# HBioquant/DiffBindFR

Hardware: AMD Instinct MI355X
Metric: poses_per_sec (higher is better)
Workload: dtype f32

## Files before the change

### diffbindfr_amd/csrc/convz.hip

```cpp
#include <cstdio>
#include <cstdlib>
#include <type_traits>

#include "common.h"

typedef float f32x4 __attribute__((ext_vector_type(4)));
typedef float f32x2 __attribute__((ext_vector_type(2)));
typedef _Float16 f16x8 __attribute__((ext_vector_type(8)));
typedef _Float16 f16x4 __attribute__((ext_vector_type(4)));
typedef _Float16 f16x2 __attribute__((ext_vector_type(2)));
typedef unsigned u32x4 __attribute__((ext_vector_type(4)));
typedef unsigned u32x2 __attribute__((ext_vector_type(2)));

#define CH_TILE_BYTES 9280
#define CH_TAIL_OFF 8192
#define CH_BIAS_OFF 9216

#define CZ_VSTRIDE 2064
#define CZ_CB (8 * CZ_VSTRIDE)
#define CZ_NCB 2
#define CZ_TILE (CZ_NCB * CZ_CB)
#define CZ_KPB 1
#define CZ_BUF (CZ_KPB * CZ_TILE)
#define CZ_ZBYTES (2 * CZ_BUF)
#define CZ_NHL 2
#define CZ_WAVE_FLOATS (32 * 12 + 32 + 32 + 32 + 32 + 32 + CZ_MAXSEG * 16 + 24 * 64 + CZ_NHL * 256)
#ifndef CZ_PRIO
#define CZ_PRIO 1
#endif
#if CZ_PRIO
#define CZ_SETPRIO(x) __builtin_amdgcn_s_setprio(x)
#else
#define CZ_SETPRIO(x)
#endif
#ifndef CZ_FETCH_AT
#define CZ_FETCH_AT 4
#endif
#ifndef CZ_PF_KT
#define CZ_PF_KT 7
#endif
#define CZ_ZSCALE (-20)

__device__ __forceinline__ void cz_split2(float x0, float x1, unsigned& hi, unsigned& lo) {
  const f16x2 h = __builtin_convertvector((f32x2){x0, x1}, f16x2);
  const f16x2 l = __builtin_convertvector((f32x2){x0 - (float)h[0], x1 - (float)h[1]}, f16x2);
  hi = __builtin_bit_cast(unsigned, h);
  lo = __builtin_bit_cast(unsigned, l);
}
__device__ __forceinline__ float cz_wave_max(float v) {
#pragma unroll
  for (int o = 1; o < 64; o <<= 1) v = fmaxf(v, __shfl_xor(v, o));
  return v;
}

__device__ __forceinline__ int cz_lane_here() {
  int l = __builtin_amdgcn_mbcnt_hi(~0u, __builtin_amdgcn_mbcnt_lo(~0u, 0u));
  asm volatile("" : "+v"(l));
  return l;
}

template <int I, int N, typename F>
__device__ __forceinline__ void cz_static_for(F&& f) {
  if constexpr (I < N) { f(std::integral_constant<int, I>{}); cz_static_for<I + 1, N>(f); }
}

template <int NW, int ABL = 0>
__global__ __launch_bounds__(64 * NW, 2) void k_convz(ConvZArgs a) {
  constexpr int KT = 9;
  extern __shared__ __attribute__((aligned(16))) float lds[];
  const int tid = threadIdx.x, lane = tid & 63, wave = __builtin_amdgcn_readfirstlane(tid >> 6);
  const int n = lane & 15, g = lane >> 4;
  char* zb = reinterpret_cast<char*>(lds);
  float* wl = lds + CZ_ZBYTES / 4 + wave * CZ_WAVE_FLOATS;
  float* w_sh = wl;
  float* w_sa = wl + 32 * 12;
  float* w_ua = w_sa + 32;
  int* w_row = reinterpret_cast<int*>(w_ua + 32);
  int* w_seg = w_row + 32;
  int* w_first = w_seg + 32;
  unsigned* w_mask = reinterpret_cast<unsigned*>(w_first + 32);
  float* w_xs = reinterpret_cast<float*>(w_mask + CZ_MAXSEG * 16);
  u32x4* w_hl = reinterpret_cast<u32x4*>(w_xs + 24 * 64);
  int* b_nseg = reinterpret_cast<int*>(lds + CZ_ZBYTES / 4 + NW * CZ_WAVE_FLOATS);
  int* b_col_edge = b_nseg + NW;
  float* b_col_inv = reinterpret_cast<float*>(b_col_edge + 16 * CZ_NCB);
  unsigned* b_cdesc = reinterpret_cast<unsigned*>(b_col_inv + 16 * CZ_NCB);

  int tr_n = 0;
  auto stamp = [&](int tag) {
    if constexpr ((ABL & 128) != 0) {
      if (a.dbg && blockIdx.x == 0 && lane == 0 && tr_n < 1000) {
        unsigned long long* t = reinterpret_cast<unsigned long long*>(a.dbg) + wave * 1024;
        t[tr_n++] = (__builtin_amdgcn_s_memtime() << 8) | (unsigned)tag;
      }
    }
  };
  int nch[4] = {0, 0, 0, 0}, nu[4] = {0, 0, 0, 0};
#pragma unroll
  for (int c = 0; c < 4; ++c)
    if (c < a.n_conv) {
      const ConvZDesc& d = a.c[c];
      nch[c] = min(*d.n_chunks, d.max_chunks);
      nu[c] = (nch[c] + NW - 1) / NW;
    }
  const int N = nu[0] + nu[1] + nu[2] + nu[3];
  for (int unit = blockIdx.x; unit < N; unit += gridDim.x) {
    int c = 0, ul = unit;
    if (ul >= nu[0]) { ul -= nu[0]; c = 1; if (ul >= nu[1]) { ul -= nu[1]; c = 2; if (ul >= nu[2]) { ul -= nu[2]; c = 3; } } }
    const ConvZDesc& d = a.c[c];
    const ConvZ& W = d.w;
    const int E = min(*d.n_edges, d.max_edges);
    unsigned cd_t = 0u;
    if (tid < (W.ct0[W.n_io - 1] + W.nct[W.n_io - 1]) * 16) cd_t = W.cdesc[tid];
    const int ch = ul * NW + wave;
    int es = 0, len = 0, gidx = 0;
    if (ch < nch[c]) {
      es = d.chunk_es[ch];
      const int gl = d.chunk_gl[ch];
      gidx = gl >> 6;
      len = min(min(gl & 63, 32), max(E - es, 0));
    }
    __syncthreads();
    if (unit != (int)blockIdx.x) tr_n = 1000;
    stamp(1);
    const int sl = lane & 31;
    const bool have = len > 0;
    const int e_sl = have ? es + min(sl, len - 1) : 0;
    const int tgt_ld = d.tgt[e_sl], gth_ld = d.gth[e_sl];
    float s_l[9];
    {
      const float* sp = d.sh + (size_t)e_sl * SH_LD;
#pragma unroll
      for (int k = 0; k < 9; ++k) s_l[k] = sp[k];
    }
    const float xmax_g = d.xmax ? d.xmax[gidx] : 0.f;
    int i1_t[2], i2_t[2];
    f32x4 Ba_t[2][9];
#pragma unroll
    for (int et = 0; et < 2; ++et) {
      const int e = have ? es + min(16 * et + n, len - 1) : 0;
      i1_t[et] = d.idx1[e];
      i2_t[et] = d.idx2[e];
      const float* r0 = d.emb + (size_t)e * NS;
#pragma unroll
      for (int s4 = 0; s4 < 3; ++s4) Ba_t[et][s4] = *reinterpret_cast<const f32x4*>(r0 + 16 * s4 + 4 * g);
    }
    const int tgt_l = have ? tgt_ld : 0, gth_l = have ? gth_ld : 0;
    const int tgt_prev = __shfl_up(tgt_l, 1);
    const bool is_first = lane < 32 && sl < len && (sl == 0 || tgt_l != tgt_prev);
    const unsigned long long bal = __ballot(is_first);
    const unsigned firsts = (unsigned)bal;
    const int nseg = min(__popc(firsts), CZ_MAXSEG);
    const int seg_l = (sl < len) ? __popc(firsts & (0xffffffffu >> (31 - sl))) - 1 : -1;
    if (lane < 32) {
      w_row[sl] = gth_l * d.ldx;
      w_seg[sl] = seg_l;
      if (is_first) w_first[seg_l] = sl;
#pragma unroll
      for (int k = 0; k < 9; ++k) w_sh[sl * 12 + k] = have ? s_l[k] : 0.f;
      w_sh[sl * 12 + 9] = w_sh[sl * 12 + 10] = w_sh[sl * 12 + 11] = 0.f;
    }
    if (lane == 0) b_nseg[wave] = nseg;
    if (tid < CZ_MAXCT * 16) b_cdesc[tid] = cd_t;
    float xmx = 0.f, smx = 0.f;
    if (have) {
      if (d.xmax) xmx = xmax_g;
      else {
        const float* xr = d.x + (size_t)gth_l * d.ldx;
        const int d4 = d.ldx >> 2;
        for (int j = lane >> 5; j < d4; j += 2) {
          const f32x4 v = *reinterpret_cast<const f32x4*>(xr + 4 * j);
          xmx = fmaxf(fmaxf(xmx, fmaxf(fabsf(v[0]), fabsf(v[1]))), fmaxf(fabsf(v[2]), fabsf(v[3])));
        }
      }
      if (lane < 32) {
#pragma unroll
        for (int k = 0; k < 9; ++k) smx = fmaxf(smx, fabsf(s_l[k]));
      }
    }
    xmx = cz_wave_max(xmx); smx = cz_wave_max(smx);
    int ey = 0;
    if (xmx > 0.f && smx > 0.f) ey = max(-100, min(100, 13 - __builtin_amdgcn_frexp_expf(xmx) - __builtin_amdgcn_frexp_expf(smx)));
    ey = __builtin_amdgcn_readfirstlane(ey);
    const float sY = __builtin_amdgcn_ldexpf(1.f, ey);

    stamp(2);
    u32x4 Hh[CZ_NKT][2];
    int eh = 0;
    {
      const __amdgpu_buffer_rsrc_t rW1 = __builtin_amdgcn_make_buffer_rsrc((void*)W.W1h, 0, KT * CH_TILE_BYTES, 0x00020000);
      u32x4 Ah[2][2][4];
      u32x4 Atc[2];
      const int vW = lane * 16;
      u32x4 F[3][2];
      auto ldF = [&](auto ic) {
        constexpr int i = decltype(ic)::value, m = i / 5, sx = i % 5;
        if constexpr (sx < 4) {
          F[i % 3][0] = __builtin_bit_cast(u32x4, __builtin_amdgcn_raw_buffer_load_b128(rW1, vW, m * CH_TILE_BYTES + sx * 1024, 0));
          F[i % 3][1] = __builtin_bit_cast(u32x4, __builtin_amdgcn_raw_buffer_load_b128(rW1, vW, m * CH_TILE_BYTES + (4 + sx) * 1024, 0));
        } else {
          F[i % 3][0] = __builtin_bit_cast(u32x4, __builtin_amdgcn_raw_buffer_load_b128(rW1, vW, m * CH_TILE_BYTES + CH_TAIL_OFF, 0));
          F[i % 3][1][0] = __builtin_amdgcn_raw_buffer_load_b32(rW1, n * 4, m * CH_TILE_BYTES + CH_BIAS_OFF, 0);
        }
      };
#pragma unroll
      for (int et = 0; et < 2; ++et) {
        const float* r1 = d.tab1 + (size_t)i1_t[et] * d.ld1;
        const float* r2 = d.tab2 + (size_t)i2_t[et] * d.ld2;
#pragma unroll
        for (int s4 = 3; s4 < KT; ++s4) Ba_t[et][s4] = *reinterpret_cast<const f32x4*>((s4 < 6 ? r1 : r2) + 16 * (s4 % 3) + 4 * g);
      }
      ldF(std::integral_constant<int, 0>{});
      ldF(std::integral_constant<int, 1>{});
#pragma unroll
      for (int et = 0; et < 2; ++et) {
        const int slot = 16 * et + n;
        f32x4 Ba[KT];
        float amx = 0.f;
#pragma unroll
        for (int s4 = 0; s4 < KT; ++s4) {
          Ba[s4] = have ? Ba_t[et][s4] : (f32x4){0.f, 0.f, 0.f, 0.f};
#pragma unroll
          for (int q = 0; q < 4; ++q) amx = fmaxf(amx, fabsf(Ba[s4][q]));
        }
        amx = fmaxf(amx, __shfl_xor(amx, 16));
        amx = fmaxf(amx, __shfl_xor(amx, 32));
        const int ja = max(-14, __builtin_amdgcn_frexp_expf(amx));
        const float sa = __builtin_amdgcn_ldexpf(1.f, 15 - ja);
        if (g == 0) { w_sa[slot] = sa; w_ua[slot] = __builtin_amdgcn_ldexpf(1.f, ja - 15); }
#pragma unroll
        for (int s4 = 0; s4 < KT; ++s4) {
          unsigned hi0, lo0, hi1, lo1;
          cz_split2(Ba[s4][0] * sa, Ba[s4][1] * sa, hi0, lo0);
          cz_split2(Ba[s4][2] * sa, Ba[s4][3] * sa, hi1, lo1);
          if (s4 < 8) {
            Ah[et][0][s4 >> 1][2 * (s4 & 1)] = hi0; Ah[et][0][s4 >> 1][2 * (s4 & 1) + 1] = hi1;
            Ah[et][1][s4 >> 1][2 * (s4 & 1)] = lo0; Ah[et][1][s4 >> 1][2 * (s4 & 1) + 1] = lo1;
          } else {
            Atc[et] = (u32x4){lo0, lo1, hi0, hi1};
          }
        }
      }
      __builtin_amdgcn_wave_barrier();
      f32x4 sar[2], uar[2];
#pragma unroll
      for (int et = 0; et < 2; ++et) {
        sar[et] = *reinterpret_cast<const f32x4*>(w_sa + 16 * et + 4 * g);
        uar[et] = *reinterpret_cast<const f32x4*>(w_ua + 16 * et + 4 * g);
      }
      float Hf[KT][2][4];
      float hmx = 0.f;
      f32x4 acc[2];
      cz_static_for<0, 5 * KT>([&](auto ic) {
        constexpr int i = decltype(ic)::value, m = i / 5, sx = i % 5;
        if constexpr (i + 2 < 5 * KT) ldF(std::integral_constant<int, (i + 2 < 5 * KT ? i + 2 : 0)>{});
        if constexpr (sx == 0) { acc[0] = (f32x4){0.f, 0.f, 0.f, 0.f}; acc[1] = (f32x4){0.f, 0.f, 0.f, 0.f}; }
        if constexpr (sx < 4) {
          const f16x8 whi = __builtin_bit_cast(f16x8, F[i % 3][0]), wlo = __builtin_bit_cast(f16x8, F[i % 3][1]);
#pragma unroll
          for (int et = 0; et < 2; ++et) {
            acc[et] = __builtin_amdgcn_mfma_f32_16x16x32_f16(__builtin_bit_cast(f16x8, Ah[et][1][sx]), whi, acc[et], 0, 0, 0);
            acc[et] = __builtin_amdgcn_mfma_f32_16x16x32_f16(__builtin_bit_cast(f16x8, Ah[et][0][sx]), wlo, acc[et], 0, 0, 0);
            acc[et] = __builtin_amdgcn_mfma_f32_16x16x32_f16(__builtin_bit_cast(f16x8, Ah[et][0][sx]), whi, acc[et], 0, 0, 0);
          }
        } else {
          const u32x4 wt = F[i % 3][0];
          const f16x8 wf = __builtin_bit_cast(f16x8, wt);
          const f16x8 wh = __builtin_bit_cast(f16x8, (u32x4){wt[0], wt[1], 0u, 0u});
          const float bias = __builtin_bit_cast(float, F[i % 3][1][0]);
          const float w1r = W.W1rinv ? W.W1rinv[16 * m + n] : 1.f;
#pragma unroll
          for (int et = 0; et < 2; ++et) {
            acc[et] = __builtin_amdgcn_mfma_f32_16x16x32_f16(__builtin_bit_cast(f16x8, Atc[et]), wf, acc[et], 0, 0, 0);
            acc[et] = __builtin_amdgcn_mfma_f32_16x16x32_f16(__builtin_bit_cast(f16x8, (u32x4){Atc[et][2], Atc[et][3], 0u, 0u}), wh, acc[et], 0, 0, 0);
          }
#pragma unroll
          for (int et = 0; et < 2; ++et)
#pragma unroll
            for (int q = 0; q < 4; ++q) {
              const float v = fmaxf(acc[et][q] + bias * sar[et][q], 0.f) * (uar[et][q] * w1r);
              Hf[m][et][q] = v;
              hmx = fmaxf(hmx, v);
            }
        }
      });
      if (!(ABL & 128) && a.dbg && unit == 0 && wave == 0) {
        const float k1i = __builtin_amdgcn_ldexpf(1.f, -W.k1);
#pragma unroll
        for (int m = 0; m < KT; ++m)
#pragma unroll
          for (int et = 0; et < 2; ++et)
#pragma unroll
            for (int q = 0; q < 4; ++q) a.dbg[(16 * et + 4 * g + q) * 144 + 16 * m + n] = Hf[m][et][q] * k1i;
      }
      hmx = cz_wave_max(hmx);
      eh = max(hmx > 0.f ? __builtin_amdgcn_frexp_expf(hmx) : W.k1, W.k1);
      eh = min(eh, W.k1 + 100);
      const float sH = __builtin_amdgcn_ldexpf(1.f, 15 - eh);
#pragma unroll
      for (int m = 0; m < KT; ++m) {
        unsigned h0, l0, h1, l1, h2, l2, h3, l3;
        cz_split2(Hf[m][0][0] * sH, Hf[m][0][1] * sH, h0, l0);
        cz_split2(Hf[m][0][2] * sH, Hf[m][0][3] * sH, h1, l1);
        cz_split2(Hf[m][1][0] * sH, Hf[m][1][1] * sH, h2, l2);
        cz_split2(Hf[m][1][2] * sH, Hf[m][1][3] * sH, h3, l3);
        Hh[m][0] = (u32x4){h0, h1, h2, h3};
        if (m < CZ_NHL) w_hl[m * 64 + lane] = (u32x4){l0, l1, l2, l3};
        else Hh[m][1] = (u32x4){l0, l1, l2, l3};
      }
    }
    const int ephi = 15 - eh + W.k1;
    {
      const _Float16 ph = (_Float16)__builtin_amdgcn_ldexpf(1.f, ephi);
      const unsigned short pb = __builtin_bit_cast(unsigned short, ph);
      u32x4 hb = {0u, 0u, 0u, 0u};
      if (n == 0) {
#pragma unroll
        for (int t = 0; t < 8; ++t) {
          const int slot = t < 4 ? 4 * g + t : 16 + 4 * g + (t - 4);
          if (slot < len) hb[t >> 1] |= (unsigned)pb << (16 * (t & 1));
        }
      }
      Hh[KT][0] = hb;
      Hh[KT][1] = (u32x4){0u, 0u, 0u, 0u};
    }
    stamp(3);
    {
      const int j = lane >> 4, gg = (lane >> 2) & 3, r = lane & 3, t0 = 2 * r;
      const int s0 = t0 < 4 ? 4 * gg + t0 : 16 + 4 * gg + (t0 - 4);
      w_mask[lane] = (w_seg[s0] == j ? 0x0000ffffu : 0u) | (w_seg[s0 + 1] == j ? 0xffff0000u : 0u);
    }
    __builtin_amdgcn_wave_barrier();
    __syncthreads();
    int cbase = 0, total = 0;
#pragma unroll
    for (int v = 0; v < NW; ++v) { const int c = b_nseg[v]; if (v < wave) cbase += c; total += c; }
    cbase = __builtin_amdgcn_readfirstlane(cbase); total = __builtin_amdgcn_readfirstlane(total);
    const int nseg_u = __builtin_amdgcn_readfirstlane(nseg);
    const int ncb = (total + 15) >> 4;
    const float col_inv = __builtin_amdgcn_ldexpf(1.f, -CZ_ZSCALE - ey - ephi);
    const float zs = __builtin_amdgcn_ldexpf(1.f, CZ_ZSCALE);
    if (ABL & 32) continue;
    for (int c = tid; c < 16 * CZ_NCB; c += 64 * NW) b_col_edge[c] = -1;
    __syncthreads();
    if (lane < nseg_u) {
      b_col_edge[cbase + lane] = es + w_first[lane];
      b_col_inv[cbase + lane] = col_inv;
    }
    char* za[CZ_MAXSEG];
    {
      char* zw0 = zb + (n & 7) * CZ_VSTRIDE + g * 512 + (n >> 3) * 256;
#pragma unroll
      for (int j = 0; j < CZ_MAXSEG; ++j) {
        const int col = cbase + j;
        za[j] = j < nseg_u ? zw0 + (col >> 4) * CZ_CB + (col & 15) * 16 : zw0 + CZ_CB + 15 * 16;
      }
    }
    long long n_mfma = 2 * KT * 14;
    for (int io = 0; io < W.n_io; ++io) {
      n_mfma += (long long)W.nct[io] * (3LL * CZ_NKT * CZ_MAXSEG + 9LL * ncb * (KT + (wave == 0)));
      f32x4 acc[3][CZ_NCB];
#pragma unroll
      for (int wt = 0; wt < 3; ++wt)
#pragma unroll
        for (int cb = 0; cb < CZ_NCB; ++cb) acc[wt][cb] = (f32x4){0.f, 0.f, 0.f, 0.f};
      const char* wbase = reinterpret_cast<const char*>(W.W2z) + (size_t)lane * 16;
      int gq = W.ct0[io] * CZ_NKT;
      const int gq_last = (W.ct0[io] + W.nct[io]) * CZ_NKT - 1;
      u32x4 Wf[2][3][2];
      auto fetchW = [&](auto par_c, int q, int share) {
        constexpr int par = decltype(par_c)::value;
        if ((ABL & 1) && q != W.ct0[io] * CZ_NKT) return;
        const char* p = wbase + ((size_t)q * 8 + share) * CZ_TILE_BYTES;
#pragma unroll
        for (int wt = 0; wt < 3; ++wt)
#pragma unroll
          for (int pc = 0; pc < 2; ++pc) Wf[par][wt][pc] = *reinterpret_cast<const u32x4*>(p + (wt * 2 + pc) * 1024);
      };
      u32x4 Ym[CZ_MAXSEG][2];
#pragma unroll
      for (int j = 0; j < CZ_MAXSEG; ++j) { Ym[j][0] = (u32x4){0u, 0u, 0u, 0u}; Ym[j][1] = (u32x4){0u, 0u, 0u, 0u}; }
      auto prefetch_x = [&](int ct) {
        if (nseg_u == 0 || (ABL & 16)) return;
        const int lane = __builtin_amdgcn_mbcnt_hi(~0u, __builtin_amdgcn_mbcnt_lo(~0u, 0u)), n = lane & 15, g = lane >> 4;
        const unsigned cd_n = b_cdesc[(W.ct0[io] + ct) * 16 + n];
        const bool vec = (__builtin_amdgcn_readfirstlane(cd_n) >> 12) & 1u;
        const int xo = cd_n & 0xfff;
        const unsigned lds0 = (unsigned)(size_t)(const void __attribute__((address_space(3)))*)w_xs;
#pragma unroll
        for (int t = 0; t < 8; ++t) {
          const float* xp = d.x + w_row[t < 4 ? 4 * g + t : 16 + 4 * g + (t - 4)] + xo;
          asm volatile("s_mov_b32 m0, %0\n\ts_nop 0\n\tglobal_load_lds_dword %1, off" ::"s"(__builtin_amdgcn_readfirstlane(lds0 + t * 256)), "v"(xp) : "memory");
          if (vec) {
            asm volatile("s_mov_b32 m0, %0\n\ts_nop 0\n\tglobal_load_lds_dword %1, off" ::"s"(__builtin_amdgcn_readfirstlane(lds0 + (8 + t) * 256)), "v"(xp + 1) : "memory");
            asm volatile("s_mov_b32 m0, %0\n\ts_nop 0\n\tglobal_load_lds_dword %1, off" ::"s"(__builtin_amdgcn_readfirstlane(lds0 + (16 + t) * 256)), "v"(xp + 2) : "memory");
          }
        }
      };
      auto wait_stage = [&](auto younger_c) {
        constexpr int y = decltype(younger_c)::value;
        static_assert(y == 0 || y == 6, "wait_stage: a fetch is six loads");
        __builtin_amdgcn_sched_barrier(0);
        if constexpr (y == 0) asm volatile("s_waitcnt vmcnt(0)" ::: "memory");
        else asm volatile("s_waitcnt vmcnt(6)" ::: "memory");
        __builtin_amdgcn_sched_barrier(0);
      };
      auto finish_Y = [&](int ct) {
        if (nseg_u == 0 || (ABL & 16)) return;
        const int lane = cz_lane_here(), n = lane & 15, g = lane >> 4;
        const unsigned cd_n = b_cdesc[(W.ct0[io] + ct) * 16 + n];
        const bool vec = (__builtin_amdgcn_readfirstlane(cd_n) >> 12) & 1u;
        const int so = (cd_n >> 16) & 15;
        const float yv = (cd_n >> 31) ? sY : 0.f;
        float y[8];
        if (!vec) {
          float xs[8], s0[8];
#pragma unroll
          for (int t = 0; t < 8; ++t) { xs[t] = w_xs[t * 64 + lane]; s0[t] = w_sh[(t < 4 ? 4 * g + t : 16 + 4 * g + (t - 4)) * 12 + so]; }
#pragma unroll
          for (int t = 0; t < 8; ++t) y[t] = xs[t] * s0[t] * yv;
        } else {
          float xs[8][3], s1[8][3];
#pragma unroll
          for (int t = 0; t < 8; ++t)
#pragma unroll
            for (int m = 0; m < 3; ++m) { xs[t][m] = w_xs[(8 * m + t) * 64 + lane]; s1[t][m] = w_sh[(t < 4 ? 4 * g + t : 16 + 4 * g + (t - 4)) * 12 + so + m]; }
#pragma unroll
          for (int t = 0; t < 8; ++t) y[t] = (xs[t][0] * s1[t][0] + xs[t][1] * s1[t][1] + xs[t][2] * s1[t][2]) * yv;
        }
        u32x4 Yh, Yl;
#pragma unroll
        for (int r = 0; r < 4; ++r) { unsigned hi, lo; cz_split2(y[2 * r], y[2 * r + 1], hi, lo); Yh[r] = hi; Yl[r] = lo; }
#pragma unroll
        for (int j = 0; j < CZ_MAXSEG; ++j) {
          const u32x4 mk = *reinterpret_cast<const u32x4*>(w_mask + (j * 4 + g) * 4);
          Ym[j][0] = Yh & mk; Ym[j][1] = Yl & mk;
        }
      };
#define YM(j, p) __builtin_bit_cast(f16x8, Ym[j][p])
#define MF(a, b, c) __builtin_amdgcn_mfma_f32_16x16x32_f16(a, b, c, 0, 0, 0)
#define SL __builtin_amdgcn_sched_barrier(0)
      auto load_hl = [&](auto kt_c) -> u32x4 {
        constexpr int kt = decltype(kt_c)::value;
        if constexpr (kt < CZ_NHL) {
          return w_hl[kt * 64 + cz_lane_here()];
        } else
          return Hh[kt][1];
      };
      auto stepA = [&](auto kt_c, auto buf_c) {
        constexpr int kt = decltype(kt_c)::value, boff = decltype(buf_c)::value * CZ_BUF;
        if (ABL & 4) return;
        const f32x4 zero = {0.f, 0.f, 0.f, 0.f};
        const f16x8 hh = __builtin_bit_cast(f16x8, Hh[kt][0]), hl = __builtin_bit_cast(f16x8, load_hl(kt_c));
        f32x4 z[CZ_MAXSEG];
#pragma unroll
        for (int j = 0; j < CZ_MAXSEG; ++j) z[j] = MF(YM(j, 0), hl, zero);
#pragma unroll
        for (int j = 0; j < CZ_MAXSEG; ++j) z[j] = MF(YM(j, 1), hh, z[j]);
#pragma unroll
        for (int j = 0; j < CZ_MAXSEG; ++j) z[j] = MF(YM(j, 0), hh, z[j]);
#pragma unroll
        for (int j = 0; j < CZ_MAXSEG; ++j) *reinterpret_cast<f32x4*>(za[j] + boff) = z[j];
      };
      auto cut = [&](const f32x4 (&zf)[2], u32x4& zh, u32x4& zl, auto r_c) {
        constexpr int r = decltype(r_c)::value;
        unsigned hi, lo;
        cz_split2(zf[r >> 1][2 * (r & 1)] * zs, zf[r >> 1][2 * (r & 1) + 1] * zs, hi, lo);
        zh[r] = hi; zl[r] = lo;
      };
      using K0 = std::integral_constant<int, 0>; using K1 = std::integral_constant<int, 1>;
      using K2 = std::integral_constant<int, 2>; using K3 = std::integral_constant<int, 3>;
      auto tile = [&](auto kt_c, auto ncb_c) {
        constexpr int kt = decltype(kt_c)::value, NCBV = decltype(ncb_c)::value;
        constexpr int boffA = ((kt + 1) & 1) * CZ_BUF;
        if constexpr (CZ_FETCH_AT == 0) fetchW(std::integral_constant<int, (kt + 1) & 1>{}, min(gq + 1, gq_last), kt + 1 == KT ? 0 : wave);
        const char* zr = zb + (kt & 1) * CZ_BUF + wave * CZ_VSTRIDE + g * 512 + n * 16;
        f32x4 zf0[2], zf1[2];
        zf0[0] = *reinterpret_cast<const f32x4*>(zr); zf0[1] = *reinterpret_cast<const f32x4*>(zr + 256);
        const f32x4 zero = {0.f, 0.f, 0.f, 0.f};
        const f16x8 hh = __builtin_bit_cast(f16x8, Hh[kt + 1][0]), hl = __builtin_bit_cast(f16x8, load_hl(std::integral_constant<int, kt + 1>{}));
        u32x4 p0h, p0l, p1h, p1l;
        f32x4 z0, z1, z2, z3;
        if constexpr ((ABL & 4) != 0) {
          z0 = z1 = z2 = z3 = zero;
          cut(zf0, p0h, p0l, K0{}); cut(zf0, p0h, p0l, K1{}); cut(zf0, p0h, p0l, K2{}); cut(zf0, p0h, p0l, K3{});
        } else {
        CZ_SETPRIO(3);
        SL;
        z0 = MF(YM(0, 0), hl, zero); SL;
        z1 = MF(YM(1, 0), hl, zero); SL;
        z2 = MF(YM(2, 0), hl, zero); SL;
        z3 = MF(YM(3, 0), hl, zero); SL;
        if constexpr (CZ_FETCH_AT == 4) { fetchW(std::integral_constant<int, (kt + 1) & 1>{}, min(gq + 1, gq_last), kt + 1 == KT ? 0 : wave); SL; }
        z0 = MF(YM(0, 1), hh, z0); cut(zf0, p0h, p0l, K0{}); SL;
        z1 = MF(YM(1, 1), hh, z1); SL;
        z2 = MF(YM(2, 1), hh, z2); cut(zf0, p0h, p0l, K1{}); SL;
        z3 = MF(YM(3, 1), hh, z3); SL;
        if constexpr (CZ_FETCH_AT == 8) { fetchW(std::integral_constant<int, (kt + 1) & 1>{}, min(gq + 1, gq_last), kt + 1 == KT ? 0 : wave); SL; }
        CZ_SETPRIO(2);
        z0 = MF(YM(0, 0), hh, z0); cut(zf0, p0h, p0l, K2{}); SL;
        z1 = MF(YM(1, 0), hh, z1); SL;
        z2 = MF(YM(2, 0), hh, z2); cut(zf0, p0h, p0l, K3{}); SL;
        z3 = MF(YM(3, 0), hh, z3); SL;
        if constexpr (CZ_FETCH_AT == 12) { fetchW(std::integral_constant<int, (kt + 1) & 1>{}, min(gq + 1, gq_last), kt + 1 == KT ? 0 : wave); SL; }
        }
        if constexpr ((ABL & 4) != 0 && CZ_FETCH_AT != 0) fetchW(std::integral_constant<int, (kt + 1) & 1>{}, min(gq + 1, gq_last), kt + 1 == KT ? 0 : wave);
#define WFR(wt, pc) __builtin_bit_cast(f16x8, Wf[kt & 1][wt][pc])
        if constexpr ((ABL & 8) != 0) {
          if constexpr (!(ABL & 4)) { *reinterpret_cast<f32x4*>(za[0] + boffA) = z0; *reinterpret_cast<f32x4*>(za[1] + boffA) = z1; *reinterpret_cast<f32x4*>(za[2] + boffA) = z2; *reinterpret_cast<f32x4*>(za[3] + boffA) = z3; }
          asm volatile("" :: "v"(p0h), "v"(p0l));
        } else {
          const f16x8 zh = __builtin_bit_cast(f16x8, p0h), zl = __builtin_bit_cast(f16x8, p0l);
          if constexpr (NCBV > 1) { zf1[0] = *reinterpret_cast<const f32x4*>(zr + CZ_CB); zf1[1] = *reinterpret_cast<const f32x4*>(zr + CZ_CB + 256); }
          acc[0][0] = MF(WFR(0, 0), zl, acc[0][0]); *reinterpret_cast<f32x4*>(za[0] + boffA) = z0; SL;
          acc[1][0] = MF(WFR(1, 0), zl, acc[1][0]); *reinterpret_cast<f32x4*>(za[1] + boffA) = z1; SL;
          acc[2][0] = MF(WFR(2, 0), zl, acc[2][0]); *reinterpret_cast<f32x4*>(za[2] + boffA) = z2; SL;
          acc[0][0] = MF(WFR(0, 1), zh, acc[0][0]); *reinterpret_cast<f32x4*>(za[3] + boffA) = z3; SL;
          CZ_SETPRIO(1);
          acc[1][0] = MF(WFR(1, 1), zh, acc[1][0]); if constexpr (NCBV > 1) cut(zf1, p1h, p1l, K0{}); SL;
          acc[2][0] = MF(WFR(2, 1), zh, acc[2][0]); if constexpr (NCBV > 1) cut(zf1, p1h, p1l, K1{}); SL;
          acc[0][0] = MF(WFR(0, 0), zh, acc[0][0]); if constexpr (NCBV > 1) cut(zf1, p1h, p1l, K2{}); SL;
          acc[1][0] = MF(WFR(1, 0), zh, acc[1][0]); if constexpr (NCBV > 1) cut(zf1, p1h, p1l, K3{}); SL;
          acc[2][0] = MF(WFR(2, 0), zh, acc[2][0]); SL;
        }
        if constexpr (NCBV > 1 && !(ABL & 8)) {
          const f16x8 zh = __builtin_bit_cast(f16x8, p1h), zl = __builtin_bit_cast(f16x8, p1l);
          acc[0][1] = MF(WFR(0, 0), zl, acc[0][1]); SL;
          acc[1][1] = MF(WFR(1, 0), zl, acc[1][1]); SL;
          acc[2][1] = MF(WFR(2, 0), zl, acc[2][1]); SL;
          CZ_SETPRIO(0);
          acc[0][1] = MF(WFR(0, 1), zh, acc[0][1]); SL;
          acc[1][1] = MF(WFR(1, 1), zh, acc[1][1]); SL;
          acc[2][1] = MF(WFR(2, 1), zh, acc[2][1]); SL;
          acc[0][1] = MF(WFR(0, 0), zh, acc[0][1]); SL;
          acc[1][1] = MF(WFR(1, 0), zh, acc[1][1]); SL;
          acc[2][1] = MF(WFR(2, 0), zh, acc[2][1]); SL;
        }
      };
      auto tile9 = [&](int ct) {
        constexpr int kt = KT;
        fetchW(K0{}, min(gq + 1, gq_last), wave);
        wait_stage(std::integral_constant<int, 6>{});
        if (wave == 0 && !(ABL & 8)) {
          const int lane = cz_lane_here(), n = lane & 15, g = lane >> 4;
          const char* zr = zb + (kt & 1) * CZ_BUF + g * 512 + n * 16;
#pragma unroll
          for (int cb = 0; cb < CZ_NCB; ++cb)
            if (cb < ncb) {
              f32x4 zf[2];
              zf[0] = *reinterpret_cast<const f32x4*>(zr + cb * CZ_CB); zf[1] = *reinterpret_cast<const f32x4*>(zr + cb * CZ_CB + 256);
              u32x4 ph, pl;
              cut(zf, ph, pl, K0{}); cut(zf, ph, pl, K1{}); cut(zf, ph, pl, K2{}); cut(zf, ph, pl, K3{});
              const f16x8 zh = __builtin_bit_cast(f16x8, ph), zl = __builtin_bit_cast(f16x8, pl);
#pragma unroll
              for (int wt = 0; wt < 3; ++wt) {
                acc[wt][cb] = MF(WFR(wt, 0), zl, acc[wt][cb]);
                acc[wt][cb] = MF(WFR(wt, 1), zh, acc[wt][cb]);
                acc[wt][cb] = MF(WFR(wt, 0), zh, acc[wt][cb]);
              }
            }
        }
        if (ct + 1 < W.nct[io]) { finish_Y(ct + 1); stepA(K0{}, K0{}); }
      };
#undef WFR
      prefetch_x(0);
      wait_stage(K0{});
      auto run_tiles = [&](auto ncb_c) {
        fetchW(K0{}, gq, wave);
        finish_Y(0);
        stepA(K0{}, K0{});
        __syncthreads();
        for (int ct = 0; ct < W.nct[io]; ++ct) {
          cz_static_for<0, CZ_NKT>([&](auto kt_c) {
            constexpr int kt = decltype(kt_c)::value;
            stamp(10);
            if constexpr (kt < KT) {
              tile(kt_c, ncb_c);
              if constexpr (kt == CZ_PF_KT) if (ct + 1 < W.nct[io]) prefetch_x(ct + 1);
            } else
              tile9(ct);
            stamp(12);
            ++gq;
            if (!(ABL & 2)) __syncthreads();
            stamp(13);
          });
        }
      };
      if (ncb > 1) run_tiles(K2{}); else run_tiles(K1{});
#undef YM
#undef MF
#undef SL
      float* red = reinterpret_cast<float*>(zb) + wave * (12 * CZ_NCB * 64);
#pragma unroll
      for (int wt = 0; wt < 3; ++wt)
#pragma unroll
        for (int cb = 0; cb < CZ_NCB; ++cb)
#pragma unroll
          for (int q = 0; q < 4; ++q) red[((wt * CZ_NCB + cb) * 4 + q) * 64 + lane] = acc[wt][cb][q];
      __syncthreads();
      for (int idx = tid; idx < 16 * ncb * 48; idx += 64 * NW) {
        const int col = idx / 48, w = idx - 48 * col;
        const int e = b_col_edge[col];
        if (e >= 0) {
          const int r = w & 15;
          const float* rp = reinterpret_cast<const float*>(zb) + (((w >> 4) * CZ_NCB + (col >> 4)) * 4 + (r & 3)) * 64 + 16 * (r >> 2) + (col & 15);
          float s = 0.f;
#pragma unroll
          for (int v = 0; v < NW; ++v) s += rp[v * (12 * CZ_NCB * 64)];
          d.msg[(size_t)e * d.D_out + W.out_off[io] + w] = s * b_col_inv[col] * W.rowinv[io * 48 + w];
        }
      }
      __syncthreads();
    }
    if (a.executed && lane == 0) atomicAdd(a.executed, 16384.0 * (double)n_mfma);
  }
}

__global__ void k_convz_useful(ConvZArgs a) {
  for (int c = 0; c < a.n_conv; ++c) {
    const ConvZDesc& d = a.c[c];
    const ConvZ& W = d.w;
    const int nch = min(*d.n_chunks, d.max_chunks), E = min(*d.n_edges, d.max_edges);
    double useful = 0.0, bytes = 0.0;
    for (int ch = blockIdx.x * blockDim.x + threadIdx.x; ch < nch; ch += gridDim.x * blockDim.x) {
      const int es = d.chunk_es[ch], len = min(min(d.chunk_gl[ch] & 63, 32), max(E - es, 0));
      int nseg = 0;
      for (int i = 0; i < len; ++i) nseg += (i == 0 || d.tgt[es + i] != d.tgt[es + i - 1]);
      nseg = min(nseg, CZ_MAXSEG);
      double u = 144.0 * 144.0 * len;
      for (int io = 0; io < W.n_io; ++io) u += (double)W.nc_valid[io] * 145.0 * ((double)len + 48.0 * nseg);
      useful += 6.0 * u;
      bytes += 4.0 * 48.0 * W.n_io * nseg;
    }
    if (useful > 0.0) { atomicAdd(a.executed + 1, useful); atomicAdd(a.executed + 2, bytes); }
  }
}

size_t convz_lds_bytes() { return CZ_ZBYTES + 8 * CZ_WAVE_FLOATS * sizeof(float) + (8 + 2 * 16 * CZ_NCB + CZ_MAXCT * 16) * sizeof(int); }

void launch_convz(const ConvZArgs& a0, hipStream_t st) {
  constexpr int NW = 8;
  ConvZArgs a = a0;
  static float* dbg_dev = nullptr;
  static const char* dbg_file = getenv("DBFR_CONVZ_DEBUG");
  if (dbg_file && !dbg_dev) {
    if (hipMalloc(&dbg_dev, 8 * 1024 * 8) != hipSuccess || hipMemset(dbg_dev, 0, 8 * 1024 * 8) != hipSuccess) dbg_dev = nullptr;
    else atexit([] {
      std::vector<float> h(8 * 1024 * 2);
      if (hipDeviceSynchronize() == hipSuccess && hipMemcpy(h.data(), dbg_dev, h.size() * 4, hipMemcpyDeviceToHost) == hipSuccess)
        if (FILE* f = fopen(getenv("DBFR_CONVZ_DEBUG"), "wb")) { fwrite(h.data(), 4, h.size(), f); fclose(f); }
    });
  }
  a.dbg = dbg_dev;
  const size_t lds = convz_lds_bytes();
#define V(x) { if (dbfr_launch_check(hipFuncSetAttribute(reinterpret_cast<const void*>(&k_convz<NW, x>), hipFuncAttributeMaxDynamicSharedMemorySize, (int)lds), "k_convz: hipFuncSetAttribute(MaxDynamicSharedMemorySize)")) return; \
               hipLaunchKernelGGL((k_convz<NW, x>), dim3(dbfr_current_cu_count()), dim3(64 * NW), lds, st, a); return; }
#ifdef DBFR_DEV_VARIANTS
  static int abl = getenv("DBFR_CONVZ_ABL") ? atoi(getenv("DBFR_CONVZ_ABL")) : 0;
  if (abl == 1) V(1) if (abl == 2) V(2) if (abl == 4) V(4) if (abl == 8) V(8) if (abl == 16) V(16) if (abl == 32) V(32) if (abl == 12) V(12) if (abl == 5) V(5) if (abl == 64) V(64) if (abl == 128) V(128)
#endif
  if (a.executed) hipLaunchKernelGGL(k_convz_useful, dim3(64), dim3(256), 0, st, a);
  V(0)
#undef V
}
```

Baseline: 512.2.

## Issue first x gather early and pipeline weight/x prefetch across io groups

Moves the first x-row gather for the initial column tile much earlier, right after edge metadata is staged, so its latency overlaps the xmax/scale computations. It also restructures the io loop into a single run_unit lambda with a shared gq counter and weight registers, so the prefetch for the next io group's first tile is issued during the previous group's tiles instead of stalling at each io start. This adds complexity in waitcnt accounting (a hand-coded s_waitcnt value) and a risk of mismatched prefetch indices across io boundaries.

```diff
diff --git a/diffbindfr_amd/csrc/convz.hip b/diffbindfr_amd/csrc/convz.hip
--- a/diffbindfr_amd/csrc/convz.hip
+++ b/diffbindfr_amd/csrc/convz.hip
@@ -134,6 +134,7 @@
       for (int k = 0; k < 9; ++k) s_l[k] = sp[k];
     }
     const float xmax_g = d.xmax ? d.xmax[gidx] : 0.f;
+    const unsigned cd_first = W.cdesc[W.ct0[0] * 16 + n];
     int i1_t[2], i2_t[2];
     f32x4 Ba_t[2][9];
 #pragma unroll
@@ -162,6 +163,23 @@
     }
     if (lane == 0) b_nseg[wave] = nseg;
     if (tid < CZ_MAXCT * 16) b_cdesc[tid] = cd_t;
+    auto gather_x = [&](unsigned cd_n) {
+      const int g = __builtin_amdgcn_mbcnt_hi(~0u, __builtin_amdgcn_mbcnt_lo(~0u, 0u)) >> 4;
+      const bool vec = (__builtin_amdgcn_readfirstlane(cd_n) >> 12) & 1u;
+      const int xo = cd_n & 0xfff;
+      const unsigned lds0 = (unsigned)(size_t)(const void __attribute__((address_space(3)))*)w_xs;
+#pragma unroll
+      for (int t = 0; t < 8; ++t) {
+        const float* xp = d.x + w_row[t < 4 ? 4 * g + t : 16 + 4 * g + (t - 4)] + xo;
+        asm volatile("s_mov_b32 m0, %0\n\ts_nop 0\n\tglobal_load_lds_dword %1, off" ::"s"(__builtin_amdgcn_readfirstlane(lds0 + t * 256)), "v"(xp) : "memory");
+        if (vec) {
+          asm volatile("s_mov_b32 m0, %0\n\ts_nop 0\n\tglobal_load_lds_dword %1, off" ::"s"(__builtin_amdgcn_readfirstlane(lds0 + (8 + t) * 256)), "v"(xp + 1) : "memory");
+          asm volatile("s_mov_b32 m0, %0\n\ts_nop 0\n\tglobal_load_lds_dword %1, off" ::"s"(__builtin_amdgcn_readfirstlane(lds0 + (16 + t) * 256)), "v"(xp + 2) : "memory");
+        }
+      }
+    };
+    __builtin_amdgcn_wave_barrier();
+    if (__builtin_amdgcn_readfirstlane(nseg) != 0 && !(ABL & 16)) gather_x(cd_first);
     float xmx = 0.f, smx = 0.f;
     if (have) {
       if (d.xmax) xmx = xmax_g;
@@ -357,6 +375,11 @@
       }
     }
     long long n_mfma = 2 * KT * 14;
+    auto run_unit = [&](auto ncb_c) {
+    u32x4 Wf[2][3][2];
+    const int io_last = W.n_io - 1;
+    const int gq_last = (W.ct0[io_last] + W.nct[io_last]) * CZ_NKT - 1;
+    int gq = W.ct0[0] * CZ_NKT;
     for (int io = 0; io < W.n_io; ++io) {
       n_mfma += (long long)W.nct[io] * (3LL * CZ_NKT * CZ_MAXSEG + 9LL * ncb * (KT + (wave == 0)));
       f32x4 acc[3][CZ_NCB];
@@ -365,12 +388,9 @@
 #pragma unroll
         for (int cb = 0; cb < CZ_NCB; ++cb) acc[wt][cb] = (f32x4){0.f, 0.f, 0.f, 0.f};
       const char* wbase = reinterpret_cast<const char*>(W.W2z) + (size_t)lane * 16;
-      int gq = W.ct0[io] * CZ_NKT;
-      const int gq_last = (W.ct0[io] + W.nct[io]) * CZ_NKT - 1;
-      u32x4 Wf[2][3][2];
       auto fetchW = [&](auto par_c, int q, int share) {
         constexpr int par = decltype(par_c)::value;
-        if ((ABL & 1) && q != W.ct0[io] * CZ_NKT) return;
+        if ((ABL & 1) && q != W.ct0[0] * CZ_NKT) return;
         const char* p = wbase + ((size_t)q * 8 + share) * CZ_TILE_BYTES;
 #pragma unroll
         for (int wt = 0; wt < 3; ++wt)
@@ -382,20 +402,8 @@
       for (int j = 0; j < CZ_MAXSEG; ++j) { Ym[j][0] = (u32x4){0u, 0u, 0u, 0u}; Ym[j][1] = (u32x4){0u, 0u, 0u, 0u}; }
       auto prefetch_x = [&](int ct) {
         if (nseg_u == 0 || (ABL & 16)) return;
-        const int lane = __builtin_amdgcn_mbcnt_hi(~0u, __builtin_amdgcn_mbcnt_lo(~0u, 0u)), n = lane & 15, g = lane >> 4;
-        const unsigned cd_n = b_cdesc[(W.ct0[io] + ct) * 16 + n];
-        const bool vec = (__builtin_amdgcn_readfirstlane(cd_n) >> 12) & 1u;
-        const int xo = cd_n & 0xfff;
-        const unsigned lds0 = (unsigned)(size_t)(const void __attribute__((address_space(3)))*)w_xs;
-#pragma unroll
-        for (int t = 0; t < 8; ++t) {
-          const float* xp = d.x + w_row[t < 4 ? 4 * g + t : 16 + 4 * g + (t - 4)] + xo;
-          asm volatile("s_mov_b32 m0, %0\n\ts_nop 0\n\tglobal_load_lds_dword %1, off" ::"s"(__builtin_amdgcn_readfirstlane(lds0 + t * 256)), "v"(xp) : "memory");
-          if (vec) {
-            asm volatile("s_mov_b32 m0, %0\n\ts_nop 0\n\tglobal_load_lds_dword %1, off" ::"s"(__builtin_amdgcn_readfirstlane(lds0 + (8 + t) * 256)), "v"(xp + 1) : "memory");
-            asm volatile("s_mov_b32 m0, %0\n\ts_nop 0\n\tglobal_load_lds_dword %1, off" ::"s"(__builtin_amdgcn_readfirstlane(lds0 + (16 + t) * 256)), "v"(xp + 2) : "memory");
-          }
-        }
+        const int n = __builtin_amdgcn_mbcnt_hi(~0u, __builtin_amdgcn_mbcnt_lo(~0u, 0u)) & 15;
+        gather_x(b_cdesc[(W.ct0[io] + ct) * 16 + n]);
       };
       auto wait_stage = [&](auto younger_c) {
         constexpr int y = decltype(younger_c)::value;
@@ -563,30 +571,32 @@
         if (ct + 1 < W.nct[io]) { finish_Y(ct + 1); stepA(K0{}, K0{}); }
       };
 #undef WFR
-      prefetch_x(0);
-      wait_stage(K0{});
-      auto run_tiles = [&](auto ncb_c) {
+      if (io == 0) {
+        wait_stage(K0{});
         fetchW(K0{}, gq, wave);
-        finish_Y(0);
-        stepA(K0{}, K0{});
-        __syncthreads();
-        for (int ct = 0; ct < W.nct[io]; ++ct) {
-          cz_static_for<0, CZ_NKT>([&](auto kt_c) {
-            constexpr int kt = decltype(kt_c)::value;
-            stamp(10);
-            if constexpr (kt < KT) {
-              tile(kt_c, ncb_c);
-              if constexpr (kt == CZ_PF_KT) if (ct + 1 < W.nct[io]) prefetch_x(ct + 1);
-            } else
-              tile9(ct);
-            stamp(12);
-            ++gq;
-            if (!(ABL & 2)) __syncthreads();
-            stamp(13);
-          });
-        }
-      };
-      if (ncb > 1) run_tiles(K2{}); else run_tiles(K1{});
+      } else {
+        __builtin_amdgcn_sched_barrier(0);
+        __builtin_amdgcn_s_waitcnt(0x0f70);
+        __builtin_amdgcn_sched_barrier(0);
+      }
+      finish_Y(0);
+      stepA(K0{}, K0{});
+      __syncthreads();
+      for (int ct = 0; ct < W.nct[io]; ++ct) {
+        cz_static_for<0, CZ_NKT>([&](auto kt_c) {
+          constexpr int kt = decltype(kt_c)::value;
+          stamp(10);
+          if constexpr (kt < KT) {
+            tile(kt_c, ncb_c);
+            if constexpr (kt == CZ_PF_KT) if (ct + 1 < W.nct[io] || io + 1 < W.n_io) prefetch_x(ct + 1);
+          } else
+            tile9(ct);
+          stamp(12);
+          ++gq;
+          if (!(ABL & 2)) __syncthreads();
+          stamp(13);
+        });
+      }
 #undef YM
 #undef MF
 #undef SL
@@ -612,6 +622,8 @@
       }
       __syncthreads();
     }
+    };
+    if (ncb > 1) run_unit(std::integral_constant<int, 2>{}); else run_unit(std::integral_constant<int, 1>{});
     if (a.executed && lane == 0) atomicAdd(a.executed, 16384.0 * (double)n_mfma);
   }
 }
```

Measured after the change: 470.8. 8.1% lower.
